# UCSD-Comp-Imaging/Nerf-Simple

Measured on AMD Instinct MI355X. Metric: ray-samples/sec at 800x800x128, higher is better.
Workload: dtype f16

## Files before the change

### nerf-simple_amd/csrc/dw_gemm.hip

```cpp
#include "nerf_device.h"

using namespace nerf_layout;

typedef __bf16 bf16x4 __attribute__((ext_vector_type(4)));

namespace {

constexpr int MAXD = 16;
struct GemmDesc {
    const __bf16* A;
    const __bf16* B;
    float* C;
    int lda, ldb, ldc;
    int M, N;
    int r0, Mv, Nv;
    int wg0, wgs;
    float* bias;
};
struct GemmTable {
    GemmDesc d[MAXD];
    int n;
    long long P;
};

constexpr int SLAB = 32;
static_assert(SLAB == 32, "the slab loop is written for two k-steps");
static_assert(ACT_TILE_PTS % SLAB == 0 && ACT_TILE_PTS * 16 == 4096, "a slab never straddles activation blocks");
constexpr int ROWB = 512;
constexpr int OPB = SLAB * ROWB;
constexpr int KSTEP = 16 * ROWB;
constexpr int SLOTB = 2 * OPB;
constexpr int RING = 4;
constexpr int LDS_BYTES = RING * SLOTB;
constexpr int DMA_PER_SLAB = 2 * SLAB / 2 / 8;

struct Frag { bf16x4 lo, hi; };
template <int KOFF>
__device__ __forceinline__ void read_frag_tr(Frag& f, unsigned addr_lo, unsigned addr_hi) {
    asm volatile("ds_read_b64_tr_b16 %0, %2 offset:%4\n\tds_read_b64_tr_b16 %1, %3 offset:%4"
                 : "=&v"(f.lo), "=&v"(f.hi) : "v"(addr_lo), "v"(addr_hi), "n"(KOFF));
}
__device__ __forceinline__ void frags_landed(Frag (&a)[4], Frag (&b)[2]) {
    asm volatile("s_waitcnt lgkmcnt(0)"
                 : "+v"(a[0].lo), "+v"(a[0].hi), "+v"(a[1].lo), "+v"(a[1].hi), "+v"(a[2].lo), "+v"(a[2].hi),
                   "+v"(a[3].lo), "+v"(a[3].hi), "+v"(b[0].lo), "+v"(b[0].hi), "+v"(b[1].lo), "+v"(b[1].hi));
}
__device__ __forceinline__ bf16x8 whole(const Frag& f) {
    return bf16x8{f.lo[0], f.lo[1], f.lo[2], f.lo[3], f.hi[0], f.hi[1], f.hi[2], f.hi[3]};
}

__global__ __launch_bounds__(512, 2) void dw_gemm_kernel(GemmTable tab) {
    extern __shared__ __attribute__((aligned(16))) char smem[];
    int di = 0;
    while (di + 1 < tab.n && (int)blockIdx.x >= tab.d[di + 1].wg0) ++di;
    const GemmDesc d = tab.d[di];
    const int slice = blockIdx.x - d.wg0;
    const long long nslab = (tab.P + SLAB - 1) / SLAB;
    const long long s_begin = nslab * slice / d.wgs, s_end = nslab * (slice + 1) / d.wgs;

    const int tid = threadIdx.x, lane = tid & 63;
    const int wave = __builtin_amdgcn_readfirstlane(tid >> 6);
    const int wm = wave >> 2, wn = wave & 3;
    const int m0 = 128 * wm, n0 = 64 * wn;

    const bool pieceA = wave < 4;
    const int pld = pieceA ? d.lda : d.ldb;
    const bool pblk = pld == 0;
    const __bf16* pbase = pieceA ? d.A : d.B;
    const int pwidth = pieceA ? d.M : d.N;
    const long long row_begin = s_begin * SLAB;
    const long long row_end = s_end * SLAB < tab.P ? s_end * SLAB : tab.P;
    const long long slice_rows = row_end > row_begin ? row_end - row_begin : 0;
    const long long slice_blocks = (row_end + ACT_TILE_PTS - 1) / ACT_TILE_PTS - row_begin / ACT_TILE_PTS;
    const __amdgpu_buffer_rsrc_t rs = pblk
        ? __builtin_amdgcn_make_buffer_rsrc(const_cast<char*>(reinterpret_cast<const char*>(pbase))
                                                + (row_begin / ACT_TILE_PTS) * ACT_BLOCK_BYTES,
                                            0, (int)(slice_rows > 0 ? slice_blocks * ACT_BLOCK_BYTES : 0), 0x00020000)
        : __builtin_amdgcn_make_buffer_rsrc(const_cast<__bf16*>(pbase + row_begin * pld), 0,
                                            (int)(slice_rows * pld * 2), 0x00020000);
    constexpr unsigned OUTSIDE = 0xffffffffu;
    unsigned voff[DMA_PER_SLAB];
    unsigned ldst[DMA_PER_SLAB];
    int vrow[DMA_PER_SLAB];
#pragma unroll
    for (int k = 0; k < DMA_PER_SLAB; ++k) {
        const int piece = wave * DMA_PER_SLAB + k, pi = piece & 15;
        ldst[k] = (piece >> 4) * OPB + pi * 1024;
        if (pblk) {
            const int c = 4 * (pi & 7) + (lane >> 4);
            vrow[k] = 16 * (pi >> 3) + ((lane & 15) ^ ((lane >> 4) << 2));
            voff[k] = c * 8 < pwidth ? (unsigned)(c * (ACT_TILE_PTS * 16) + vrow[k] * 16) : OUTSIDE;
        } else {
            vrow[k] = 2 * pi + (lane >> 5);
            const int cg = (lane & 31) ^ ((vrow[k] & 3) << 2);
            voff[k] = cg * 8 < pwidth ? (unsigned)(vrow[k] * pld * 2 + cg * 16) : OUTSIDE;
        }
    }
    auto issue_slab = [&](int it, int slot) {
        const long long p0 = row_begin + (long long)it * SLAB;
        unsigned vadd;
        int rows_left = SLAB;
        if (pblk) {
            vadd = (unsigned)((p0 / ACT_TILE_PTS - row_begin / ACT_TILE_PTS) * ACT_BLOCK_BYTES + (p0 % ACT_TILE_PTS) * 16);
            rows_left = tab.P - p0 < SLAB ? (int)(tab.P - p0) : SLAB;
        } else {
            vadd = (unsigned)it * (unsigned)(SLAB * pld * 2);
        }
#pragma unroll
        for (int k = 0; k < DMA_PER_SLAB; ++k) {
            lds_void* dst = reinterpret_cast<lds_void*>(reinterpret_cast<lds_char*>(0) + slot * SLOTB + ldst[k]);
            const unsigned off = (voff[k] == OUTSIDE || vrow[k] >= rows_left) ? OUTSIDE : voff[k] + vadd;
            __builtin_amdgcn_raw_ptr_buffer_load_lds(rs, dst, 16, off, 0, 0, 2);
        }
    };

    const int grp = lane >> 4, q = (lane & 15) >> 2, pp = lane & 3, h = lane >> 5;
    const int cl = 2 * (grp & 1) + (pp >> 1);
    auto frag_addr = [&](bool blocked, int t, int second) -> unsigned {
        const int r = 8 * h + q + 4 * second;
        if (blocked) return (4 * t + cl) * 256 + ((r ^ (cl << 2)) * 16) + 8 * (pp & 1);
        return r * ROWB + ((((4 * t + cl) ^ ((r & 3) << 2))) * 16) + 8 * (pp & 1);
    };
    unsigned aoff[4][2], boff[2][2];
#pragma unroll
    for (int i = 0; i < 4; ++i)
#pragma unroll
        for (int e = 0; e < 2; ++e) aoff[i][e] = frag_addr(d.lda == 0, m0 / 32 + i, e);
#pragma unroll
    for (int j = 0; j < 2; ++j)
#pragma unroll
        for (int e = 0; e < 2; ++e) boff[j][e] = OPB + frag_addr(d.ldb == 0, n0 / 32 + j, e);

    f32x16 acc[4][2];
#pragma unroll
    for (int i = 0; i < 4; ++i)
#pragma unroll
        for (int j = 0; j < 2; ++j)
#pragma unroll
            for (int r = 0; r < 16; ++r) acc[i][j][r] = 0.f;
    const bool active = m0 < d.M && n0 < d.N;
    float bsum[8] = {0.f, 0.f, 0.f, 0.f, 0.f, 0.f, 0.f, 0.f};
    const int brow = tid & 15, bchunk = tid >> 4;
    const unsigned baddr = bchunk * 256 + ((brow ^ ((bchunk & 3) << 2)) * 16);

#pragma unroll
    for (int k = 0; k < RING - 1; ++k)
        if (s_begin + k < s_end) issue_slab(k, k);
    Frag a0[4], b0[2], a1[4], b1[2];
    auto read_k0 = [&](unsigned base) {
#pragma unroll
        for (int i = 0; i < 4; ++i) read_frag_tr<0>(a0[i], base + aoff[i][0], base + aoff[i][1]);
#pragma unroll
        for (int j = 0; j < 2; ++j) read_frag_tr<0>(b0[j], base + boff[j][0], base + boff[j][1]);
    };
    if (s_begin < s_end) {
        const long long n = s_end - s_begin;
        if (n >= 3) asm volatile("s_waitcnt vmcnt(8)" ::: "memory");
        else if (n == 2) asm volatile("s_waitcnt vmcnt(4)" ::: "memory");
        else asm volatile("s_waitcnt vmcnt(0)" ::: "memory");
        __builtin_amdgcn_s_barrier();
        if (active) read_k0(0);
    }
    for (long long s = s_begin; s < s_end; ++s) {
        const int it = (int)(s - s_begin), slot = it & (RING - 1);
        const long long left = s_end - s;
        const unsigned base = slot * SLOTB;
        if (active) {
            frags_landed(a0, b0);
#pragma unroll
            for (int i = 0; i < 4; ++i) read_frag_tr<KSTEP>(a1[i], base + aoff[i][0], base + aoff[i][1]);
#pragma unroll
            for (int j = 0; j < 2; ++j) read_frag_tr<KSTEP>(b1[j], base + boff[j][0], base + boff[j][1]);
            __builtin_amdgcn_sched_barrier(0);
#pragma unroll
            for (int i = 0; i < 4; ++i)
#pragma unroll
                for (int j = 0; j < 2; ++j)
                    acc[i][j] = __builtin_amdgcn_mfma_f32_32x32x16_bf16(whole(a0[i]), whole(b0[j]), acc[i][j], 0, 0, 0);
            __builtin_amdgcn_sched_barrier(0);
        }
        if (left >= 2) {
            if (left >= 3) asm volatile("s_waitcnt vmcnt(4)" ::: "memory");
            else asm volatile("s_waitcnt vmcnt(0)" ::: "memory");
            __builtin_amdgcn_s_barrier();
            if (s + RING - 1 < s_end) issue_slab(it + RING - 1, (it + RING - 1) & (RING - 1));
        }
        if (active) {
            frags_landed(a1, b1);
            if (left >= 2) read_k0(((it + 1) & (RING - 1)) * SLOTB);
            __builtin_amdgcn_sched_barrier(0);
#pragma unroll
            for (int i = 0; i < 4; ++i)
#pragma unroll
                for (int j = 0; j < 2; ++j)
                    acc[i][j] = __builtin_amdgcn_mfma_f32_32x32x16_bf16(whole(a1[i]), whole(b1[j]), acc[i][j], 0, 0, 0);
        }
        if (d.bias && bchunk * 8 < d.M) {
#pragma unroll
            for (int ks = 0; ks < SLAB / 16; ++ks) {
                const bf16x8 v = *reinterpret_cast<const __attribute__((address_space(3))) bf16x8*>(
                    reinterpret_cast<lds_char*>(0) + base + ks * KSTEP + baddr);
#pragma unroll
                for (int k = 0; k < 8; ++k) bsum[k] += (float)v[k];
            }
        }
    }
    __syncthreads();
    if (d.bias && bchunk * 8 < d.M && s_begin < s_end) {
        float* red = reinterpret_cast<float*>(smem);
#pragma unroll
        for (int k = 0; k < 8; ++k) red[(brow * 32 + bchunk) * 8 + k] = bsum[k];
    }
    __syncthreads();
    if (d.bias && s_begin < s_end && tid < d.M) {
        const int ch = tid >> 3, k = tid & 7;
        float v = 0.f;
        for (int r = 0; r < 16; ++r) v += reinterpret_cast<float*>(smem)[(r * 32 + ch) * 8 + k];
        atomicAdd(d.bias + tid, v);
    }
    if (active && s_begin < s_end) {
#pragma unroll
        for (int i = 0; i < 4; ++i)
#pragma unroll
            for (int j = 0; j < 2; ++j)
#pragma unroll
                for (int r = 0; r < 16; ++r) {
                    const int row = m0 + 32 * i + (r & 3) + 8 * (r >> 2) + 4 * h - d.r0;
                    const int col = n0 + 32 * j + (lane & 31);
                    if (row >= 0 && row < d.Mv && col < d.Nv)
                        atomicAdd(d.C + (long long)row * d.ldc + col, acc[i][j][r]);
                }
    }
}

__global__ __launch_bounds__(256) void pack_draw_kernel(const float* __restrict__ d_raw, __bf16* __restrict__ dsr,
                                                        long long P, float* __restrict__ g_rgb_b,
                                                        float* __restrict__ g_sig_b) {
    __shared__ float red[4][4];
    f32x4 s = {0.f, 0.f, 0.f, 0.f};
    const __bf16 z = (__bf16)0.f;
    for (long long p = blockIdx.x * (long long)blockDim.x + threadIdx.x; p < P; p += (long long)gridDim.x * blockDim.x) {
        const f32x4 d = *reinterpret_cast<const f32x4*>(d_raw + p * 4);
        s += d;
        bf16x8* o = reinterpret_cast<bf16x8*>(dsr + p * 32);
        o[0] = bf16x8{(__bf16)d[0], (__bf16)d[1], (__bf16)d[2], (__bf16)d[3], z, z, z, z};
        o[1] = bf16x8{z, z, z, z, z, z, z, z};
        o[2] = o[1];
        o[3] = o[1];
    }
#pragma unroll
    for (int k = 0; k < 4; ++k) {
        float v = s[k];
#pragma unroll
        for (int off = 32; off >= 1; off >>= 1) v += __shfl_xor(v, off);
        if ((threadIdx.x & 63) == 0) red[threadIdx.x >> 6][k] = v;
    }
    __syncthreads();
    if (threadIdx.x < 4) {
        const float v = red[0][threadIdx.x] + red[1][threadIdx.x] + red[2][threadIdx.x] + red[3][threadIdx.x];
        atomicAdd(threadIdx.x < 3 ? g_rgb_b + threadIdx.x : g_sig_b, v);
    }
}

__global__ __launch_bounds__(256) void zero_f32_kernel(float* __restrict__ p, long long n) {
    const long long i = (blockIdx.x * (long long)blockDim.x + threadIdx.x) * 4;
    if (i + 3 < n) *reinterpret_cast<f32x4*>(p + i) = f32x4{0.f, 0.f, 0.f, 0.f};
    else for (long long k = i; k < n; ++k) p[k] = 0.f;
}

}

extern "C" int nerf_amd_launch_param_gradients_begin(const float* d_raw, void* scratch, float* grads, long long P,
                                                     hipStream_t stream) {
    (void)hipGetLastError();
    static_assert(PARAM_COUNT % 4 == 0, "16-byte zero fill");
    hipLaunchKernelGGL(zero_f32_kernel, dim3((PARAM_COUNT / 4 + 255) / 256), dim3(256), 0, stream, grads,
                       (long long)PARAM_COUNT);
    hipError_t e = hipGetLastError();
    if (e != hipSuccess) return (int)e;
    if (P <= 0) return 0;
    hipLaunchKernelGGL(pack_draw_kernel, dim3(512), dim3(256), 0, stream, d_raw, reinterpret_cast<__bf16*>(scratch), P,
                       grads + OFF_C1_B, grads + OFF_SIG_B);
    return (int)hipGetLastError();
}

extern "C" int nerf_amd_launch_param_gradients_finish(const void* acts_v, const void* dys_v, const void* posx64_v,
                                                      const void* posd32_v, const void* scratch, float* grads,
                                                      long long P, int bucket, hipStream_t stream) {
    (void)hipGetLastError();
    hipError_t e = hipSuccess;
    if (P <= 0) return 0;
    const __bf16* acts = reinterpret_cast<const __bf16*>(acts_v);
    const __bf16* dys = reinterpret_cast<const __bf16*>(dys_v);
    const __bf16* posx = reinterpret_cast<const __bf16*>(posx64_v);
    const __bf16* posd = reinterpret_cast<const __bf16*>(posd32_v);
    const __bf16* dsr = reinterpret_cast<const __bf16*>(scratch);
    auto act = [&](int L) { return acts + act_offset_bytes(L, P) / 2; };
    auto dy = [&](int L) { return dys + act_offset_bytes(L, P) / 2; };
    constexpr int BLK = 0;

    GemmTable t{};
    t.P = P;
    int n = 0;
    auto add = [&](const __bf16* A, int lda, int M, const __bf16* B, int ldb, int N, int coff, int ldc, int r0,
                   int Mv, int Nv, int boff = -1) {
        GemmDesc& g = t.d[n++];
        g.A = A; g.lda = lda; g.M = M; g.B = B; g.ldb = ldb; g.N = N;
        g.C = grads + coff; g.ldc = ldc; g.r0 = r0; g.Mv = Mv; g.Nv = Nv;
        g.bias = boff >= 0 ? grads + boff : nullptr;
    };
    const int LW = 256 * 256 + 256;
    add(dy(0), BLK, 256, posx, 64, 64, OFF_L0_W, 63, 0, 256, 63, OFF_L0_B);
    for (int l = 1; l <= 4; ++l)
        add(dy(l), BLK, 256, act(l - 1), BLK, 256, OFF_L1_W + (l - 1) * LW, 256, 0, 256, 256,
            OFF_L1_W + (l - 1) * LW + 65536);
    add(dy(5), BLK, 256, act(4), BLK, 256, OFF_SKIP_W, 319, 0, 256, 256, OFF_SKIP_B);
    add(dy(5), BLK, 256, posx, 64, 64, OFF_SKIP_W + 256, 319, 0, 256, 63);
    add(dy(6), BLK, 256, act(5), BLK, 256, OFF_L6_W, 256, 0, 256, 256, OFF_L6_W + 65536);
    add(dy(7), BLK, 256, act(6), BLK, 256, OFF_L6_W + LW, 256, 0, 256, 256, OFF_L6_W + LW + 65536);
    add(dsr, 32, 32, act(7), BLK, 256, OFF_SIG_W, 256, 3, 1, 256);
    add(dy(8), BLK, 256, act(7), BLK, 256, OFF_L2_W, 256, 0, 256, 256, OFF_L2_B);
    add(dy(9), BLK, 128, act(8), BLK, 256, OFF_C0_W, 283, 0, 128, 256, OFF_C0_B);
    add(dy(9), BLK, 128, posd, 32, 32, OFF_C0_W + 256, 283, 0, 128, 27);
    add(dsr, 32, 32, act(9), BLK, 128, OFF_C1_W, 128, 0, 3, 128);
    if (bucket != 0) {
        int m = 0;
        for (int i = 0; i < n; ++i) {
            const bool head = t.d[i].C - grads < GRAD_BUCKET_SPLIT;
            if (head == (bucket == 2)) t.d[m++] = t.d[i];
        }
        n = m;
    }
    t.n = n;
    constexpr double slab_cost = 1024.0;
    const int cus = device_cus();
    double total = 0;
    for (int i = 0; i < n; ++i) total += (double)(t.d[i].M + t.d[i].N) + slab_cost;
    const long long nslab = (P + SLAB - 1) / SLAB;
    const long long need = (P * 512 >> 30) + 1;
    long long w[16];
    double rem[16];
    long long used = 0;
    for (int i = 0; i < n; ++i) {
        const double share = ((double)(t.d[i].M + t.d[i].N) + slab_cost) / total * cus;
        w[i] = (long long)share;
        rem[i] = share - (double)w[i];
        if (w[i] < need) { w[i] = need; rem[i] = 0; }
        if (w[i] >= nslab) { w[i] = nslab; rem[i] = -1; }
        used += w[i];
    }
    while (used < cus) {
        int best = -1;
        for (int i = 0; i < n; ++i)
            if (rem[i] >= 0 && w[i] < nslab && (best < 0 || rem[i] > rem[best])) best = i;
        if (best < 0) break;
        ++w[best]; rem[best] = 0; ++used;
    }
    int wg = 0;
    for (int i = 0; i < n; ++i) {
        t.d[i].wg0 = wg;
        t.d[i].wgs = (int)w[i];
        wg += (int)w[i];
    }
    e = allow_dynamic_lds(reinterpret_cast<const void*>(dw_gemm_kernel), LDS_BYTES);
    if (e != hipSuccess) return (int)e;
    hipLaunchKernelGGL(dw_gemm_kernel, dim3(wg), dim3(512), LDS_BYTES, stream, t);

    return (int)hipGetLastError();
}

extern "C" int nerf_amd_launch_param_gradients(const float* d_raw, const void* acts_v, const void* dys_v,
                                               const void* posx64_v, const void* posd32_v, void* scratch,
                                               float* grads, long long P, hipStream_t stream) {
    const int rc = nerf_amd_launch_param_gradients_begin(d_raw, scratch, grads, P, stream);
    if (rc) return rc;
    return nerf_amd_launch_param_gradients_finish(acts_v, dys_v, posx64_v, posd32_v, scratch, grads, P, 0, stream);
}
```

### nerf-simple_amd/csrc/dw_gemm_f8.hip

```cpp
#include "nerf_device.h"

using namespace nerf_layout;

typedef int i32x8 __attribute__((ext_vector_type(8)));
typedef int i32x2 __attribute__((ext_vector_type(2)));

namespace {

constexpr int MAXD = 16;
struct F8Operand {
    const char* data;
    const unsigned char* scales;
    int block_bytes;
    int width;
};
struct GemmDescF8 {
    F8Operand A, B;
    float* C;
    int ldc;
    int r0, Mv, Nv;
    int wg0, wgs;
    float* bias;
};
struct GemmTableF8 {
    GemmDescF8 d[MAXD];
    int n;
    long long P;
};

constexpr int SLAB = 64;
constexpr int CHS = 1152;
constexpr int OPB = 16 * CHS;
constexpr int SLOTB = 2 * OPB;
constexpr int RING = 4;
constexpr int LDS_BYTES = RING * SLOTB;
constexpr int DMA_PER_SLAB = 4;
static_assert(ACT_TILE_PTS % SLAB == 0, "a slab never straddles tiles");

typedef __attribute__((address_space(4))) const u32x4 const_u32x4;

struct Frag { i32x2 q[4]; };
__device__ __forceinline__ void read_frag(Frag& f, unsigned addr) {
    asm volatile("ds_read_b64_tr_b8 %0, %4\n\tds_read_b64_tr_b8 %1, %4 offset:128\n\t"
                 "ds_read_b64_tr_b8 %2, %4 offset:512\n\tds_read_b64_tr_b8 %3, %4 offset:640"
                 : "=&v"(f.q[0]), "=&v"(f.q[1]), "=&v"(f.q[2]), "=&v"(f.q[3]) : "v"(addr));
}
__device__ __forceinline__ void frags_landed(Frag (&a)[4], Frag (&b)[2]) {
    asm volatile("s_waitcnt lgkmcnt(0)"
                 : "+v"(a[0].q[0]), "+v"(a[0].q[1]), "+v"(a[0].q[2]), "+v"(a[0].q[3]), "+v"(a[1].q[0]), "+v"(a[1].q[1]),
                   "+v"(a[1].q[2]), "+v"(a[1].q[3]), "+v"(a[2].q[0]), "+v"(a[2].q[1]), "+v"(a[2].q[2]), "+v"(a[2].q[3]),
                   "+v"(a[3].q[0]), "+v"(a[3].q[1]), "+v"(a[3].q[2]), "+v"(a[3].q[3]), "+v"(b[0].q[0]), "+v"(b[0].q[1]),
                   "+v"(b[0].q[2]), "+v"(b[0].q[3]), "+v"(b[1].q[0]), "+v"(b[1].q[1]), "+v"(b[1].q[2]), "+v"(b[1].q[3]));
}
__device__ __forceinline__ i32x8 whole(const Frag& f) {
    return i32x8{f.q[0][0], f.q[0][1], f.q[1][0], f.q[1][1], f.q[2][0], f.q[2][1], f.q[3][0], f.q[3][1]};
}
template <int OA, int OB>
__device__ __forceinline__ void mfma(const Frag& a, const Frag& b, f32x16& c, int sa, int sb) {
    const i32x8 av = whole(a), bv = whole(b);
    static_assert(OA >= 0 && OA < 4 && OB >= 0 && OB < 4, "op_sel picks one of four exponent bytes");
    asm volatile("v_mfma_scale_f32_32x32x64_f8f6f4 %0, %1, %2, %0, %3, %4 op_sel:[%5,%6,0] op_sel_hi:[%7,%8,0]"
                 : "+v"(c) : "v"(av), "v"(bv), "v"(sa), "v"(sb), "n"(OA & 1), "n"(OB & 1), "n"(OA >> 1), "n"(OB >> 1));
}

__global__ __launch_bounds__(512, 2) void dw_gemm_e4m3_kernel(GemmTableF8 tab) {
    extern __shared__ __attribute__((aligned(16))) char smem[];
    int di = 0;
    while (di + 1 < tab.n && (int)blockIdx.x >= tab.d[di + 1].wg0) ++di;
    const GemmDescF8 d = tab.d[di];
    const int slice = blockIdx.x - d.wg0;
    const long long nslab = (tab.P + SLAB - 1) / SLAB;
    const long long s_begin = nslab * slice / d.wgs, s_end = nslab * (slice + 1) / d.wgs;

    const int tid = threadIdx.x, lane = tid & 63;
    const int wave = __builtin_amdgcn_readfirstlane(tid >> 6);
    const int wm = wave >> 2, wn = wave & 3;
    const int m0 = 128 * wm, n0 = 64 * wn;
    const int M = d.A.width, N = d.B.width;

    const bool pieceA = wave < 4;
    const F8Operand op = pieceA ? d.A : d.B;
    const long long row_begin = s_begin * SLAB;
    const long long row_end = s_end * SLAB < tab.P ? s_end * SLAB : tab.P;
    const long long slice_rows = row_end > row_begin ? row_end - row_begin : 0;
    const long long tile0 = row_begin / ACT_TILE_PTS;
    const long long slice_tiles = (row_end + ACT_TILE_PTS - 1) / ACT_TILE_PTS - tile0;
    const __amdgpu_buffer_rsrc_t rs = __builtin_amdgcn_make_buffer_rsrc(
        const_cast<char*>(op.data) + tile0 * op.block_bytes, 0, (int)(slice_rows > 0 ? slice_tiles * op.block_bytes : 0), 0x00020000);
    constexpr unsigned OUTSIDE = 0xffffffffu;
    unsigned voff[DMA_PER_SLAB], ldst[DMA_PER_SLAB];
#pragma unroll
    for (int k = 0; k < DMA_PER_SLAB; ++k) {
        const int piece = wave * DMA_PER_SLAB + k, c = piece & 15;
        ldst[k] = (piece >> 4) * OPB + c * CHS;
        voff[k] = c * 16 < op.width ? (unsigned)(c * (ACT_TILE_PTS * 16) + lane * 16) : OUTSIDE;
    }
    auto issue_slab = [&](int it, int slot) {
        const long long p0 = row_begin + (long long)it * SLAB;
        const unsigned vadd = (unsigned)((p0 / ACT_TILE_PTS - tile0) * op.block_bytes + (p0 % ACT_TILE_PTS) * 16);
        const int rows_left = tab.P - p0 < SLAB ? (int)(tab.P - p0) : SLAB;
#pragma unroll
        for (int k = 0; k < DMA_PER_SLAB; ++k) {
            lds_void* dst = reinterpret_cast<lds_void*>(reinterpret_cast<lds_char*>(0) + slot * SLOTB + ldst[k]);
            const unsigned off = (voff[k] == OUTSIDE || lane >= rows_left) ? OUTSIDE : voff[k] + vadd;
            __builtin_amdgcn_raw_ptr_buffer_load_lds(rs, dst, 16, off, 0, 0, 2);
        }
    };

    const int h = lane >> 5;
    const unsigned lane_part = (unsigned)((16 * h + ((lane & 15) >> 1)) * 16 + (lane & 1) * 8 + ((lane >> 4) & 1) * CHS);
    unsigned aoff[4], boff[2];
#pragma unroll
    for (int i = 0; i < 4; ++i) aoff[i] = (unsigned)(2 * (m0 / 32 + i) * CHS) + lane_part;
#pragma unroll
    for (int j = 0; j < 2; ++j) boff[j] = OPB + (unsigned)(2 * (n0 / 32 + j) * CHS) + lane_part;

    f32x16 acc[4][2];
#pragma unroll
    for (int i = 0; i < 4; ++i)
#pragma unroll
        for (int j = 0; j < 2; ++j)
#pragma unroll
            for (int r = 0; r < 16; ++r) acc[i][j][r] = 0.f;
    const bool active = m0 < M && n0 < N;
    bool ta[4], tb[2];
#pragma unroll
    for (int i = 0; i < 4; ++i) ta[i] = active && m0 + 32 * i < M;
#pragma unroll
    for (int j = 0; j < 2; ++j) tb[j] = active && n0 + 32 * j < N;
    unsigned amask = 0, bmask = 0;
#pragma unroll
    for (int i = 0; i < 4; ++i) amask |= (m0 + 32 * i < M) ? 0xffu << (8 * i) : 0u;
#pragma unroll
    for (int j = 0; j < 2; ++j) bmask |= (n0 + 32 * j < N) ? 0xffu << (8 * j) : 0u;

    const bool do_bias = d.bias && m0 + 32 * wn < M;
    f32x16 accb;
#pragma unroll
    for (int r = 0; r < 16; ++r) accb[r] = 0.f;
    const unsigned aoff_bias = (unsigned)(2 * (m0 / 32 + wn) * CHS) + lane_part;
    Frag ab, ones;
#pragma unroll
    for (int q = 0; q < 4; ++q) ab.q[q] = i32x2{0, 0};
#pragma unroll
    for (int q = 0; q < 4; ++q) ones.q[q] = i32x2{0x38383838, 0x38383838};

    auto load_scales = [&](long long s, u32x4& ea, u32x4& eb) {
        const long long blk = s * (SLAB / 32);
        ea = *reinterpret_cast<const_u32x4*>(reinterpret_cast<uintptr_t>(d.A.scales + blk * 8));
        eb = *reinterpret_cast<const_u32x4*>(reinterpret_cast<uintptr_t>(d.B.scales + blk * 8));
    };

#pragma unroll
    for (int k = 0; k < RING - 1; ++k)
        if (s_begin + k < s_end) issue_slab(k, k);
    u32x4 ea = {0, 0, 0, 0}, eb = {0, 0, 0, 0};
    if (s_begin < s_end) load_scales(s_begin, ea, eb);

    Frag a[4], b[2];
    for (long long s = s_begin; s < s_end; ++s) {
        const int it = (int)(s - s_begin), slot = it & (RING - 1);
        const long long left = s_end - s;
        const unsigned base = slot * SLOTB;
        if (left >= 3) asm volatile("s_waitcnt vmcnt(8)" ::: "memory");
        else if (left == 2) asm volatile("s_waitcnt vmcnt(4)" ::: "memory");
        else asm volatile("s_waitcnt vmcnt(0)" ::: "memory");
        __builtin_amdgcn_s_barrier();
        if (s + RING - 1 < s_end) issue_slab(it + RING - 1, (it + RING - 1) & (RING - 1));
        const unsigned a_dw = (h ? (wm ? ea[3] : ea[2]) : (wm ? ea[1] : ea[0])) & amask;
        const unsigned b_dw = ((h ? ((wn >> 1) ? eb[3] : eb[2]) : ((wn >> 1) ? eb[1] : eb[0])) >> (16 * (wn & 1))) & bmask;
        const u32x4 ea_now = ea;
        if (left >= 2) load_scales(s + 1, ea, eb);
#if defined(F8_TIMING) && F8_TIMING == 4
        if (false) {
#else
        if (active || do_bias) {
#endif
            if (active) {
#pragma unroll
                for (int i = 0; i < 4; ++i) read_frag(a[i], base + aoff[i]);
#pragma unroll
                for (int j = 0; j < 2; ++j) read_frag(b[j], base + boff[j]);
            }
            if (do_bias) read_frag(ab, base + aoff_bias);
            frags_landed(a, b);
            asm volatile("" : "+v"(ab.q[0]), "+v"(ab.q[1]), "+v"(ab.q[2]), "+v"(ab.q[3]));
            __builtin_amdgcn_sched_barrier(0);
            if (ta[0] && tb[0]) mfma<0, 0>(a[0], b[0], acc[0][0], (int)a_dw, (int)b_dw);
            if (ta[0] && tb[1]) mfma<0, 1>(a[0], b[1], acc[0][1], (int)a_dw, (int)b_dw);
            if (ta[1] && tb[0]) mfma<1, 0>(a[1], b[0], acc[1][0], (int)a_dw, (int)b_dw);
            if (ta[1] && tb[1]) mfma<1, 1>(a[1], b[1], acc[1][1], (int)a_dw, (int)b_dw);
            if (ta[2] && tb[0]) mfma<2, 0>(a[2], b[0], acc[2][0], (int)a_dw, (int)b_dw);
            if (ta[2] && tb[1]) mfma<2, 1>(a[2], b[1], acc[2][1], (int)a_dw, (int)b_dw);
            if (ta[3] && tb[0]) mfma<3, 0>(a[3], b[0], acc[3][0], (int)a_dw, (int)b_dw);
            if (ta[3] && tb[1]) mfma<3, 1>(a[3], b[1], acc[3][1], (int)a_dw, (int)b_dw);
#if !(defined(F8_TIMING) && F8_TIMING == 5)
            if (do_bias) {
                constexpr int ONE = 0x7f7f7f7f;
                mfma<0, 0>(ab, ones, accb, (int)(a_dw >> (8 * wn)), ONE);
            }
#endif
        }
    }
    asm volatile("s_nop 15\n\ts_nop 15" ::: "memory");
    if (do_bias && s_begin < s_end && (lane & 31) == 0) {
#pragma unroll
        for (int r = 0; r < 16; ++r) {
            const int row = m0 + 32 * wn + (r & 3) + 8 * (r >> 2) + 4 * h;
            if (row < M) atomicAdd(d.bias + row, accb[r]);
        }
    }
    if (active && s_begin < s_end) {
#pragma unroll
        for (int i = 0; i < 4; ++i)
#pragma unroll
            for (int j = 0; j < 2; ++j)
#pragma unroll
                for (int r = 0; r < 16; ++r) {
                    const int row = m0 + 32 * i + (r & 3) + 8 * (r >> 2) + 4 * h - d.r0;
                    const int col = n0 + 32 * j + (lane & 31);
                    if (row >= 0 && row < d.Mv && col < d.Nv)
                        atomicAdd(d.C + (long long)row * d.ldc + col, acc[i][j][r]);
                }
    }
}

__global__ __launch_bounds__(256) void rows_to_e4m3_kernel(const __bf16* __restrict__ src, int ld, int W, long long P,
                                                           char* __restrict__ data, unsigned char* __restrict__ scales) {
    const int lane = threadIdx.x & 63;
    const int nq = (W + 31) / 32;
    const long long nblk = (P + 31) / 32;
    const long long wid = blockIdx.x * 4ll + (threadIdx.x >> 6);
    if (wid >= nblk * nq) return;
    const long long blk = wid / nq;
    const int Q = (int)(wid - blk * nq);
    const long long p = blk * 32 + (lane & 31);
    const int c = 2 * Q + (lane >> 5);
    const bool have = p < P && c * 16 < W;
    u32x4 w0 = {0, 0, 0, 0}, w1 = {0, 0, 0, 0};
    if (have) {
        const u32x4* sp = reinterpret_cast<const u32x4*>(src + p * ld + c * 16);
        w0 = sp[0];
        w1 = sp[1];
    }
    unsigned m = 0;
#pragma unroll
    for (int k = 0; k < 4; ++k) {
        const u16x2 x = __builtin_bit_cast(u16x2, w0[k] & 0x7fff7fffu), y = __builtin_bit_cast(u16x2, w1[k] & 0x7fff7fffu);
        m = __builtin_bit_cast(unsigned, __builtin_elementwise_max(__builtin_bit_cast(u16x2, m), __builtin_elementwise_max(x, y)));
    }
    unsigned mx = (m >> 16) > (m & 0xffffu) ? (m >> 16) : (m & 0xffffu);
#pragma unroll
    for (int off = 32; off >= 1; off >>= 1) {
        const unsigned o = (unsigned)__shfl_xor((int)mx, off);
        mx = o > mx ? o : mx;
    }
    const int e = (int)(mx >> 7);
    const int sb = e > 8 ? e - 7 : 1;
    const float scale = __builtin_bit_cast(float, sb << 23);
    s16x2 t = {0, 0};
    auto cvt = [&](unsigned lo, unsigned hi) -> unsigned {
        t = __builtin_amdgcn_cvt_scalef32_pk_fp8_bf16(t, __builtin_bit_cast(bf16x2, lo), scale, false);
        t = __builtin_amdgcn_cvt_scalef32_pk_fp8_bf16(t, __builtin_bit_cast(bf16x2, hi), scale, true);
        return __builtin_bit_cast(unsigned, t);
    };
    const u32x4 o = {cvt(w0[0], w0[1]), cvt(w0[2], w0[3]), cvt(w1[0], w1[1]), cvt(w1[2], w1[3])};
    if (have)
        *reinterpret_cast<u32x4*>(data + (p / ACT_TILE_PTS) * f8_narrow_block_bytes(W) + ((long long)c * ACT_TILE_PTS + p % ACT_TILE_PTS) * 16) = o;
    if (lane == 0) scales[blk * 8 + Q] = (unsigned char)sb;
}

}

static long long align256(long long v) { return (v + 255) / 256 * 256; }
extern "C" long long nerf_amd_f8_scratch_bytes(long long P) {
    return align256(f8_narrow_bytes(64, P)) + align256(f8_narrow_bytes(32, P)) + align256(f8_narrow_bytes(16, P));
}

extern "C" int nerf_amd_launch_param_gradients_convert_e4m3(const void* posx64_v, const void* posd32_v, const void* scratch,
                                                            void* scratch_f8, long long P, int which, hipStream_t stream) {
    (void)hipGetLastError();
    if (P <= 0) return 0;
    char* px = reinterpret_cast<char*>(scratch_f8);
    char* pd = px + align256(f8_narrow_bytes(64, P));
    char* ds = pd + align256(f8_narrow_bytes(32, P));
    const long long nblk = (P + 31) / 32;
    auto convert = [&](const void* src, int ld, int W, char* dst) {
        const long long waves = nblk * ((W + 31) / 32);
        hipLaunchKernelGGL(rows_to_e4m3_kernel, dim3((unsigned)((waves + 3) / 4)), dim3(256), 0, stream,
                           reinterpret_cast<const __bf16*>(src), ld, W, P, dst,
                           reinterpret_cast<unsigned char*>(dst + f8_narrow_scale_offset(W, P)));
    };
    if (which & 1) {
        convert(posx64_v, 64, 64, px);
        convert(posd32_v, 32, 32, pd);
    }
    if (which & 2) convert(scratch, 32, 16, ds);
    return (int)hipGetLastError();
}

extern "C" int nerf_amd_launch_param_gradients_finish_e4m3(const void* acts_v, const void* dys_v, const void* scratch_f8,
                                                           float* grads, long long P, int bucket, hipStream_t stream) {
    (void)hipGetLastError();
    if (P <= 0) return 0;
    hipError_t e = hipSuccess;
    const char* acts = reinterpret_cast<const char*>(acts_v);
    const char* dys = reinterpret_cast<const char*>(dys_v);
    const char* px = reinterpret_cast<const char*>(scratch_f8);
    const char* pd = px + align256(f8_narrow_bytes(64, P));
    const char* ds = pd + align256(f8_narrow_bytes(32, P));

    auto blocked = [&](const char* buf, int L) {
        return F8Operand{buf + f8_offset_bytes(L, P), reinterpret_cast<const unsigned char*>(buf + f8_scale_offset_bytes(L, P)),
                         (int)F8_BLOCK_BYTES, act_width(L)};
    };
    auto narrow = [&](const char* buf, int W) {
        return F8Operand{buf, reinterpret_cast<const unsigned char*>(buf + f8_narrow_scale_offset(W, P)), (int)f8_narrow_block_bytes(W), W};
    };
    GemmTableF8 t{};
    t.P = P;
    int n = 0;
    auto add = [&](F8Operand A, F8Operand B, int coff, int ldc, int r0, int Mv, int Nv, int boff = -1) {
        GemmDescF8& g = t.d[n++];
        g.A = A; g.B = B; g.C = grads + coff; g.ldc = ldc; g.r0 = r0; g.Mv = Mv; g.Nv = Nv;
        g.bias = boff >= 0 ? grads + boff : nullptr;
    };
    const int LW = 256 * 256 + 256;
    add(blocked(dys, 0), narrow(px, 64), OFF_L0_W, 63, 0, 256, 63, OFF_L0_B);
    for (int l = 1; l <= 4; ++l)
        add(blocked(dys, l), blocked(acts, l - 1), OFF_L1_W + (l - 1) * LW, 256, 0, 256, 256, OFF_L1_W + (l - 1) * LW + 65536);
    add(blocked(dys, 5), blocked(acts, 4), OFF_SKIP_W, 319, 0, 256, 256, OFF_SKIP_B);
    add(blocked(dys, 5), narrow(px, 64), OFF_SKIP_W + 256, 319, 0, 256, 63);
    add(blocked(dys, 6), blocked(acts, 5), OFF_L6_W, 256, 0, 256, 256, OFF_L6_W + 65536);
    add(blocked(dys, 7), blocked(acts, 6), OFF_L6_W + LW, 256, 0, 256, 256, OFF_L6_W + LW + 65536);
    add(narrow(ds, 16), blocked(acts, 7), OFF_SIG_W, 256, 3, 1, 256);
    add(blocked(dys, 8), blocked(acts, 7), OFF_L2_W, 256, 0, 256, 256, OFF_L2_B);
    add(blocked(dys, 9), blocked(acts, 8), OFF_C0_W, 283, 0, 128, 256, OFF_C0_B);
    add(blocked(dys, 9), narrow(pd, 32), OFF_C0_W + 256, 283, 0, 128, 27);
    add(narrow(ds, 16), blocked(acts, 9), OFF_C1_W, 128, 0, 3, 128);
    if (bucket != 0) {
        int m = 0;
        for (int i = 0; i < n; ++i) {
            const bool head = t.d[i].C - grads < GRAD_BUCKET_SPLIT;
            if (head == (bucket == 2)) t.d[m++] = t.d[i];
        }
        n = m;
    }
    t.n = n;
    constexpr double slab_cost = 1024.0;
    const int cus = device_cus();
    double total = 0;
    for (int i = 0; i < n; ++i) total += (double)(t.d[i].A.width + t.d[i].B.width) + slab_cost;
    const long long nslab = (P + SLAB - 1) / SLAB;
    const long long need = (P * 256 >> 30) + 1;
    long long w[16];
    double rem[16];
    long long used = 0;
    for (int i = 0; i < n; ++i) {
        const double share = ((double)(t.d[i].A.width + t.d[i].B.width) + slab_cost) / total * cus;
        w[i] = (long long)share;
        rem[i] = share - (double)w[i];
        if (w[i] < need) { w[i] = need; rem[i] = 0; }
        if (w[i] >= nslab) { w[i] = nslab; rem[i] = -1; }
        used += w[i];
    }
    while (used < cus) {
        int best = -1;
        for (int i = 0; i < n; ++i)
            if (rem[i] >= 0 && w[i] < nslab && (best < 0 || rem[i] > rem[best])) best = i;
        if (best < 0) break;
        ++w[best]; rem[best] = 0; ++used;
    }
    int wg = 0;
    for (int i = 0; i < n; ++i) {
        t.d[i].wg0 = wg;
        t.d[i].wgs = (int)w[i];
        wg += (int)w[i];
    }
    e = allow_dynamic_lds(reinterpret_cast<const void*>(dw_gemm_e4m3_kernel), LDS_BYTES);
    if (e != hipSuccess) return (int)e;
    hipLaunchKernelGGL(dw_gemm_e4m3_kernel, dim3(wg), dim3(512), LDS_BYTES, stream, t);
    return (int)hipGetLastError();
}
```

Before: 1.366 billion.

## Merge narrow side-product weight-gradient GEMMs into their wide sibling descriptors

Folds the thin weight-gradient products (sigma head and the direction-input half of color_fc.0) into the wide GEMM that shares an operand. The shared operand is then streamed once, and an extra narrow strip is loaded per slab into a new LDS region. In the bf16 kernel a spare wave or an extra MFMA chain handles the strip; in the f8 kernel wave 4 handles it. This removes separate descriptors, their workgroups and the repeated reads of the shared operand. In exchange the LDS footprint, the per-slab DMA count and the wait counts all grow, and the kernel gets extra branching, which may cut occupancy or lengthen the critical path.

```diff
diff --git a/nerf-simple_amd/csrc/dw_gemm.hip b/nerf-simple_amd/csrc/dw_gemm.hip
--- a/nerf-simple_amd/csrc/dw_gemm.hip
+++ b/nerf-simple_amd/csrc/dw_gemm.hip
@@ -16,6 +16,10 @@
     int r0, Mv, Nv;
     int wg0, wgs;
     float* bias;
+    const __bf16* X;
+    int xside;
+    float* XC;
+    int xldc, xr0, xMv, xNv;
 };
 struct GemmTable {
     GemmDesc d[MAXD];
@@ -27,12 +31,18 @@
 static_assert(SLAB == 32, "the slab loop is written for two k-steps");
 static_assert(ACT_TILE_PTS % SLAB == 0 && ACT_TILE_PTS * 16 == 4096, "a slab never straddles activation blocks");
 constexpr int ROWB = 512;
-constexpr int OPB = SLAB * ROWB;
-constexpr int KSTEP = 16 * ROWB;
-constexpr int SLOTB = 2 * OPB;
+constexpr int HALFB = 16 * ROWB;
+constexpr int XW = 32;
+constexpr int XROWB = XW * 2;
+constexpr int XHALFB = 16 * XROWB;
+constexpr int BOFF = HALFB, XOFF = 2 * HALFB;
+constexpr int KSTEP = 2 * HALFB + XHALFB;
+constexpr int SLOTB = 2 * KSTEP;
 constexpr int RING = 4;
 constexpr int LDS_BYTES = RING * SLOTB;
-constexpr int DMA_PER_SLAB = 2 * SLAB / 2 / 8;
+constexpr int WIDE_PER_SLAB = 2 * SLAB / 2 / 8;
+constexpr int DMA_PER_SLAB = WIDE_PER_SLAB + 1;
+static_assert(KSTEP % 256 == 0 && KSTEP < 65536 && LDS_BYTES <= 160 * 1024, "ds_read offset field; LDS of a CU");
 
 struct Frag { bf16x4 lo, hi; };
 template <int KOFF>
@@ -61,7 +71,9 @@
     const int tid = threadIdx.x, lane = tid & 63;
     const int wave = __builtin_amdgcn_readfirstlane(tid >> 6);
     const int wm = wave >> 2, wn = wave & 3;
-    const int m0 = 128 * wm, n0 = 64 * wn;
+    const bool xb = d.xside == 1 && wave == 4, xa = d.xside == 2;
+    const int m0 = xb ? 0 : 128 * wm, n0 = 64 * wn;
+    const int ct[2] = {xb ? 0 : n0 / 32 + wm, xb ? 1 : n0 / 32 + (wm ^ 1)};
 
     const bool pieceA = wave < 4;
     const int pld = pieceA ? d.lda : d.ldb;
@@ -79,13 +91,13 @@
         : __builtin_amdgcn_make_buffer_rsrc(const_cast<__bf16*>(pbase + row_begin * pld), 0,
                                             (int)(slice_rows * pld * 2), 0x00020000);
     constexpr unsigned OUTSIDE = 0xffffffffu;
-    unsigned voff[DMA_PER_SLAB];
-    unsigned ldst[DMA_PER_SLAB];
-    int vrow[DMA_PER_SLAB];
-#pragma unroll
-    for (int k = 0; k < DMA_PER_SLAB; ++k) {
-        const int piece = wave * DMA_PER_SLAB + k, pi = piece & 15;
-        ldst[k] = (piece >> 4) * OPB + pi * 1024;
+    unsigned voff[WIDE_PER_SLAB];
+    unsigned ldst[WIDE_PER_SLAB];
+    int vrow[WIDE_PER_SLAB];
+#pragma unroll
+    for (int k = 0; k < WIDE_PER_SLAB; ++k) {
+        const int piece = wave * WIDE_PER_SLAB + k, pi = piece & 15;
+        ldst[k] = (pi >> 3) * KSTEP + (piece >> 4) * HALFB + (pi & 7) * 1024;
         if (pblk) {
             const int c = 4 * (pi & 7) + (lane >> 4);
             vrow[k] = 16 * (pi >> 3) + ((lane & 15) ^ ((lane >> 4) << 2));
@@ -96,6 +108,10 @@
             voff[k] = cg * 8 < pwidth ? (unsigned)(vrow[k] * pld * 2 + cg * 16) : OUTSIDE;
         }
     }
+    const __amdgpu_buffer_rsrc_t rsx = __builtin_amdgcn_make_buffer_rsrc(
+        const_cast<__bf16*>(d.X ? d.X + row_begin * XW : d.A), 0, (int)(d.X ? slice_rows * XROWB : 0), 0x00020000);
+    const unsigned xvoff = (unsigned)(wave * 4 * XROWB + lane * 16);
+    const unsigned xldst = (wave >> 2) * KSTEP + XOFF + (wave & 3) * 4 * XROWB;
     auto issue_slab = [&](int it, int slot) {
         const long long p0 = row_begin + (long long)it * SLAB;
         unsigned vadd;
@@ -107,10 +123,14 @@
             vadd = (unsigned)it * (unsigned)(SLAB * pld * 2);
         }
 #pragma unroll
-        for (int k = 0; k < DMA_PER_SLAB; ++k) {
+        for (int k = 0; k < WIDE_PER_SLAB; ++k) {
             lds_void* dst = reinterpret_cast<lds_void*>(reinterpret_cast<lds_char*>(0) + slot * SLOTB + ldst[k]);
             const unsigned off = (voff[k] == OUTSIDE || vrow[k] >= rows_left) ? OUTSIDE : voff[k] + vadd;
             __builtin_amdgcn_raw_ptr_buffer_load_lds(rs, dst, 16, off, 0, 0, 2);
+        }
+        if (lane < 16) {
+            lds_void* dst = reinterpret_cast<lds_void*>(reinterpret_cast<lds_char*>(0) + slot * SLOTB + xldst);
+            __builtin_amdgcn_raw_ptr_buffer_load_lds(rsx, dst, 16, xvoff + (unsigned)it * (unsigned)(SLAB * XROWB), 0, 0, 2);
         }
     };
 
@@ -121,7 +141,9 @@
         if (blocked) return (4 * t + cl) * 256 + ((r ^ (cl << 2)) * 16) + 8 * (pp & 1);
         return r * ROWB + ((((4 * t + cl) ^ ((r & 3) << 2))) * 16) + 8 * (pp & 1);
     };
-    unsigned aoff[4][2], boff[2][2];
+    unsigned aoff[4][2], boff[2][2], xoff[2];
+#pragma unroll
+    for (int e = 0; e < 2; ++e) xoff[e] = XOFF + (8 * h + q + 4 * e) * XROWB + cl * 16 + 8 * (pp & 1);
 #pragma unroll
     for (int i = 0; i < 4; ++i)
 #pragma unroll
@@ -129,7 +151,7 @@
 #pragma unroll
     for (int j = 0; j < 2; ++j)
 #pragma unroll
-        for (int e = 0; e < 2; ++e) boff[j][e] = OPB + frag_addr(d.ldb == 0, n0 / 32 + j, e);
+        for (int e = 0; e < 2; ++e) boff[j][e] = xb ? xoff[e] : BOFF + frag_addr(d.ldb == 0, ct[j], e);
 
     f32x16 acc[4][2];
 #pragma unroll
@@ -138,7 +160,10 @@
         for (int j = 0; j < 2; ++j)
 #pragma unroll
             for (int r = 0; r < 16; ++r) acc[i][j][r] = 0.f;
-    const bool active = m0 < d.M && n0 < d.N;
+    f32x16 accx;
+#pragma unroll
+    for (int r = 0; r < 16; ++r) accx[r] = 0.f;
+    const bool active = xb || (m0 < d.M && n0 < d.N);
     float bsum[8] = {0.f, 0.f, 0.f, 0.f, 0.f, 0.f, 0.f, 0.f};
     const int brow = tid & 15, bchunk = tid >> 4;
     const unsigned baddr = bchunk * 256 + ((brow ^ ((bchunk & 3) << 2)) * 16);
@@ -146,8 +171,10 @@
 #pragma unroll
     for (int k = 0; k < RING - 1; ++k)
         if (s_begin + k < s_end) issue_slab(k, k);
-    Frag a0[4], b0[2], a1[4], b1[2];
+    Frag a0[4], b0[2], a1[4], b1[2], ax0, ax1;
+    ax0.lo = ax0.hi = ax1.lo = ax1.hi = bf16x4{(__bf16)0.f, (__bf16)0.f, (__bf16)0.f, (__bf16)0.f};
     auto read_k0 = [&](unsigned base) {
+        if (xa) read_frag_tr<0>(ax0, base + xoff[0], base + xoff[1]);
 #pragma unroll
         for (int i = 0; i < 4; ++i) read_frag_tr<0>(a0[i], base + aoff[i][0], base + aoff[i][1]);
 #pragma unroll
@@ -155,8 +182,8 @@
     };
     if (s_begin < s_end) {
         const long long n = s_end - s_begin;
-        if (n >= 3) asm volatile("s_waitcnt vmcnt(8)" ::: "memory");
-        else if (n == 2) asm volatile("s_waitcnt vmcnt(4)" ::: "memory");
+        if (n >= 3) asm volatile("s_waitcnt vmcnt(%0)" :: "n"(2 * DMA_PER_SLAB) : "memory");
+        else if (n == 2) asm volatile("s_waitcnt vmcnt(%0)" :: "n"(DMA_PER_SLAB) : "memory");
         else asm volatile("s_waitcnt vmcnt(0)" ::: "memory");
         __builtin_amdgcn_s_barrier();
         if (active) read_k0(0);
@@ -167,6 +194,8 @@
         const unsigned base = slot * SLOTB;
         if (active) {
             frags_landed(a0, b0);
+            asm volatile("" : "+v"(ax0.lo), "+v"(ax0.hi));
+            if (xa) read_frag_tr<KSTEP>(ax1, base + xoff[0], base + xoff[1]);
 #pragma unroll
             for (int i = 0; i < 4; ++i) read_frag_tr<KSTEP>(a1[i], base + aoff[i][0], base + aoff[i][1]);
 #pragma unroll
@@ -177,16 +206,18 @@
 #pragma unroll
                 for (int j = 0; j < 2; ++j)
                     acc[i][j] = __builtin_amdgcn_mfma_f32_32x32x16_bf16(whole(a0[i]), whole(b0[j]), acc[i][j], 0, 0, 0);
+            if (xa) accx = __builtin_amdgcn_mfma_f32_32x32x16_bf16(whole(ax0), whole(b0[0]), accx, 0, 0, 0);
             __builtin_amdgcn_sched_barrier(0);
         }
         if (left >= 2) {
-            if (left >= 3) asm volatile("s_waitcnt vmcnt(4)" ::: "memory");
+            if (left >= 3) asm volatile("s_waitcnt vmcnt(%0)" :: "n"(DMA_PER_SLAB) : "memory");
             else asm volatile("s_waitcnt vmcnt(0)" ::: "memory");
             __builtin_amdgcn_s_barrier();
             if (s + RING - 1 < s_end) issue_slab(it + RING - 1, (it + RING - 1) & (RING - 1));
         }
         if (active) {
             frags_landed(a1, b1);
+            asm volatile("" : "+v"(ax1.lo), "+v"(ax1.hi));
             if (left >= 2) read_k0(((it + 1) & (RING - 1)) * SLOTB);
             __builtin_amdgcn_sched_barrier(0);
 #pragma unroll
@@ -194,6 +225,7 @@
 #pragma unroll
                 for (int j = 0; j < 2; ++j)
                     acc[i][j] = __builtin_amdgcn_mfma_f32_32x32x16_bf16(whole(a1[i]), whole(b1[j]), acc[i][j], 0, 0, 0);
+            if (xa) accx = __builtin_amdgcn_mfma_f32_32x32x16_bf16(whole(ax1), whole(b1[0]), accx, 0, 0, 0);
         }
         if (d.bias && bchunk * 8 < d.M) {
 #pragma unroll
@@ -219,17 +251,28 @@
         atomicAdd(d.bias + tid, v);
     }
     if (active && s_begin < s_end) {
+        float* const C = xb ? d.XC : d.C;
+        const int ldc = xb ? d.xldc : d.ldc, r0 = xb ? d.xr0 : d.r0, Mv = xb ? d.xMv : d.Mv, Nv = xb ? d.xNv : d.Nv;
 #pragma unroll
         for (int i = 0; i < 4; ++i)
 #pragma unroll
             for (int j = 0; j < 2; ++j)
 #pragma unroll
                 for (int r = 0; r < 16; ++r) {
-                    const int row = m0 + 32 * i + (r & 3) + 8 * (r >> 2) + 4 * h - d.r0;
-                    const int col = n0 + 32 * j + (lane & 31);
-                    if (row >= 0 && row < d.Mv && col < d.Nv)
-                        atomicAdd(d.C + (long long)row * d.ldc + col, acc[i][j][r]);
+                    const int row = m0 + 32 * i + (r & 3) + 8 * (r >> 2) + 4 * h - r0;
+                    const int col = 32 * ct[j] + (lane & 31);
+                    if (row >= 0 && row < Mv && col < Nv)
+                        atomicAdd(C + (long long)row * ldc + col, acc[i][j][r]);
                 }
+        if (xa) {
+#pragma unroll
+            for (int r = 0; r < 16; ++r) {
+                const int row = (r & 3) + 8 * (r >> 2) + 4 * h - d.xr0;
+                const int col = 32 * ct[0] + (lane & 31);
+                if (row >= 0 && row < d.xMv && col < d.xNv && col < d.N)
+                    atomicAdd(d.XC + (long long)row * d.xldc + col, accx[r]);
+            }
+        }
     }
 }
 
@@ -309,6 +352,12 @@
         g.C = grads + coff; g.ldc = ldc; g.r0 = r0; g.Mv = Mv; g.Nv = Nv;
         g.bias = boff >= 0 ? grads + boff : nullptr;
     };
+    auto merge = [&](int side, const __bf16* X, int coff, int ldc, int r0, int Mv, int Nv) {
+        GemmDesc& g = t.d[n - 1];
+        g.X = X; g.xside = side; g.XC = grads + coff; g.xldc = ldc; g.xr0 = r0; g.xMv = Mv; g.xNv = Nv;
+    };
+    static_assert(OFF_SIG_W >= GRAD_BUCKET_SPLIT && OFF_L2_W >= GRAD_BUCKET_SPLIT && OFF_C0_W >= GRAD_BUCKET_SPLIT,
+                  "layers_2 + sigma_fc.0 and both halves of color_fc.0 are late-bucket tensors");
     const int LW = 256 * 256 + 256;
     add(dy(0), BLK, 256, posx, 64, 64, OFF_L0_W, 63, 0, 256, 63, OFF_L0_B);
     for (int l = 1; l <= 4; ++l)
@@ -318,10 +367,10 @@
     add(dy(5), BLK, 256, posx, 64, 64, OFF_SKIP_W + 256, 319, 0, 256, 63);
     add(dy(6), BLK, 256, act(5), BLK, 256, OFF_L6_W, 256, 0, 256, 256, OFF_L6_W + 65536);
     add(dy(7), BLK, 256, act(6), BLK, 256, OFF_L6_W + LW, 256, 0, 256, 256, OFF_L6_W + LW + 65536);
-    add(dsr, 32, 32, act(7), BLK, 256, OFF_SIG_W, 256, 3, 1, 256);
     add(dy(8), BLK, 256, act(7), BLK, 256, OFF_L2_W, 256, 0, 256, 256, OFF_L2_B);
+    merge(2, dsr, OFF_SIG_W, 256, 3, 1, 256);
     add(dy(9), BLK, 128, act(8), BLK, 256, OFF_C0_W, 283, 0, 128, 256, OFF_C0_B);
-    add(dy(9), BLK, 128, posd, 32, 32, OFF_C0_W + 256, 283, 0, 128, 27);
+    merge(1, posd, OFF_C0_W + 256, 283, 0, 128, 27);
     add(dsr, 32, 32, act(9), BLK, 128, OFF_C1_W, 128, 0, 3, 128);
     if (bucket != 0) {
         int m = 0;
@@ -335,14 +384,15 @@
     constexpr double slab_cost = 1024.0;
     const int cus = device_cus();
     double total = 0;
-    for (int i = 0; i < n; ++i) total += (double)(t.d[i].M + t.d[i].N) + slab_cost;
+    auto width = [&](const GemmDesc& g) { return (double)(g.M + g.N + (g.X ? XW : 0)); };
+    for (int i = 0; i < n; ++i) total += width(t.d[i]) + slab_cost;
     const long long nslab = (P + SLAB - 1) / SLAB;
     const long long need = (P * 512 >> 30) + 1;
     long long w[16];
     double rem[16];
     long long used = 0;
     for (int i = 0; i < n; ++i) {
-        const double share = ((double)(t.d[i].M + t.d[i].N) + slab_cost) / total * cus;
+        const double share = (width(t.d[i]) + slab_cost) / total * cus;
         w[i] = (long long)share;
         rem[i] = share - (double)w[i];
         if (w[i] < need) { w[i] = need; rem[i] = 0; }
diff --git a/nerf-simple_amd/csrc/dw_gemm_f8.hip b/nerf-simple_amd/csrc/dw_gemm_f8.hip
--- a/nerf-simple_amd/csrc/dw_gemm_f8.hip
+++ b/nerf-simple_amd/csrc/dw_gemm_f8.hip
@@ -21,6 +21,9 @@
     int r0, Mv, Nv;
     int wg0, wgs;
     float* bias;
+    F8Operand X;
+    float* XC;
+    int xldc, xr0, xMv, xNv;
 };
 struct GemmTableF8 {
     GemmDescF8 d[MAXD];
@@ -31,10 +34,13 @@
 constexpr int SLAB = 64;
 constexpr int CHS = 1152;
 constexpr int OPB = 16 * CHS;
-constexpr int SLOTB = 2 * OPB;
+constexpr int XOFF = 2 * OPB;
+constexpr int SLOTB = 2 * OPB + 2 * CHS;
 constexpr int RING = 4;
 constexpr int LDS_BYTES = RING * SLOTB;
-constexpr int DMA_PER_SLAB = 4;
+constexpr int WIDE_PER_SLAB = 4;
+constexpr int DMA_PER_SLAB = WIDE_PER_SLAB + 1;
+static_assert(LDS_BYTES <= 160 * 1024, "LDS of a CU");
 static_assert(ACT_TILE_PTS % SLAB == 0, "a slab never straddles tiles");
 
 typedef __attribute__((address_space(4))) const u32x4 const_u32x4;
@@ -75,8 +81,10 @@
     const int tid = threadIdx.x, lane = tid & 63;
     const int wave = __builtin_amdgcn_readfirstlane(tid >> 6);
     const int wm = wave >> 2, wn = wave & 3;
-    const int m0 = 128 * wm, n0 = 64 * wn;
-    const int M = d.A.width, N = d.B.width;
+    const bool xb = d.X.data != nullptr && wave == 4;
+    const int mb = 128 * wm;
+    const int m0 = xb ? 0 : mb, n0 = 64 * wn;
+    const int M = d.A.width, N = xb ? 32 : d.B.width;
 
     const bool pieceA = wave < 4;
     const F8Operand op = pieceA ? d.A : d.B;
@@ -88,23 +96,34 @@
     const __amdgpu_buffer_rsrc_t rs = __builtin_amdgcn_make_buffer_rsrc(
         const_cast<char*>(op.data) + tile0 * op.block_bytes, 0, (int)(slice_rows > 0 ? slice_tiles * op.block_bytes : 0), 0x00020000);
     constexpr unsigned OUTSIDE = 0xffffffffu;
-    unsigned voff[DMA_PER_SLAB], ldst[DMA_PER_SLAB];
-#pragma unroll
-    for (int k = 0; k < DMA_PER_SLAB; ++k) {
-        const int piece = wave * DMA_PER_SLAB + k, c = piece & 15;
+    unsigned voff[WIDE_PER_SLAB], ldst[WIDE_PER_SLAB];
+#pragma unroll
+    for (int k = 0; k < WIDE_PER_SLAB; ++k) {
+        const int piece = wave * WIDE_PER_SLAB + k, c = piece & 15;
         ldst[k] = (piece >> 4) * OPB + c * CHS;
         voff[k] = c * 16 < op.width ? (unsigned)(c * (ACT_TILE_PTS * 16) + lane * 16) : OUTSIDE;
     }
+    const int xblock = d.X.data ? d.X.block_bytes : 0;
+    const __amdgpu_buffer_rsrc_t rsx = __builtin_amdgcn_make_buffer_rsrc(
+        const_cast<char*>(d.X.data ? d.X.data + tile0 * xblock : op.data), 0, (int)(slice_rows > 0 ? slice_tiles * xblock : 0), 0x00020000);
+    const int xpt = 16 * (wave & 3) + lane;
+    const unsigned xvoff = (unsigned)((wave >> 2) * (ACT_TILE_PTS * 16) + xpt * 16);
+    const unsigned xldst = XOFF + (wave >> 2) * CHS + (wave & 3) * 256;
     auto issue_slab = [&](int it, int slot) {
         const long long p0 = row_begin + (long long)it * SLAB;
         const unsigned vadd = (unsigned)((p0 / ACT_TILE_PTS - tile0) * op.block_bytes + (p0 % ACT_TILE_PTS) * 16);
         const int rows_left = tab.P - p0 < SLAB ? (int)(tab.P - p0) : SLAB;
 #pragma unroll
-        for (int k = 0; k < DMA_PER_SLAB; ++k) {
+        for (int k = 0; k < WIDE_PER_SLAB; ++k) {
             lds_void* dst = reinterpret_cast<lds_void*>(reinterpret_cast<lds_char*>(0) + slot * SLOTB + ldst[k]);
             const unsigned off = (voff[k] == OUTSIDE || lane >= rows_left) ? OUTSIDE : voff[k] + vadd;
             __builtin_amdgcn_raw_ptr_buffer_load_lds(rs, dst, 16, off, 0, 0, 2);
         }
+        if (lane < 16) {
+            lds_void* dst = reinterpret_cast<lds_void*>(reinterpret_cast<lds_char*>(0) + slot * SLOTB + xldst);
+            const unsigned xvadd = (unsigned)((p0 / ACT_TILE_PTS - tile0) * xblock + (p0 % ACT_TILE_PTS) * 16);
+            __builtin_amdgcn_raw_ptr_buffer_load_lds(rsx, dst, 16, xpt >= rows_left ? OUTSIDE : xvoff + xvadd, 0, 0, 2);
+        }
     };
 
     const int h = lane >> 5;
@@ -113,7 +132,7 @@
 #pragma unroll
     for (int i = 0; i < 4; ++i) aoff[i] = (unsigned)(2 * (m0 / 32 + i) * CHS) + lane_part;
 #pragma unroll
-    for (int j = 0; j < 2; ++j) boff[j] = OPB + (unsigned)(2 * (n0 / 32 + j) * CHS) + lane_part;
+    for (int j = 0; j < 2; ++j) boff[j] = (xb ? XOFF : OPB + (unsigned)(2 * (n0 / 32) * CHS)) + (unsigned)(2 * j * CHS) + lane_part;
 
     f32x16 acc[4][2];
 #pragma unroll
@@ -134,21 +153,23 @@
 #pragma unroll
     for (int j = 0; j < 2; ++j) bmask |= (n0 + 32 * j < N) ? 0xffu << (8 * j) : 0u;
 
-    const bool do_bias = d.bias && m0 + 32 * wn < M;
+    const bool do_bias = d.bias && mb + 32 * wn < M;
     f32x16 accb;
 #pragma unroll
     for (int r = 0; r < 16; ++r) accb[r] = 0.f;
-    const unsigned aoff_bias = (unsigned)(2 * (m0 / 32 + wn) * CHS) + lane_part;
+    const unsigned aoff_bias = (unsigned)(2 * (mb / 32 + wn) * CHS) + lane_part;
     Frag ab, ones;
 #pragma unroll
     for (int q = 0; q < 4; ++q) ab.q[q] = i32x2{0, 0};
 #pragma unroll
     for (int q = 0; q < 4; ++q) ones.q[q] = i32x2{0x38383838, 0x38383838};
 
+    const unsigned char* const bscales = xb ? d.X.scales : d.B.scales;
+    const int wma = xb ? 0 : wm;
     auto load_scales = [&](long long s, u32x4& ea, u32x4& eb) {
         const long long blk = s * (SLAB / 32);
         ea = *reinterpret_cast<const_u32x4*>(reinterpret_cast<uintptr_t>(d.A.scales + blk * 8));
-        eb = *reinterpret_cast<const_u32x4*>(reinterpret_cast<uintptr_t>(d.B.scales + blk * 8));
+        eb = *reinterpret_cast<const_u32x4*>(reinterpret_cast<uintptr_t>(bscales + blk * 8));
     };
 
 #pragma unroll
@@ -162,12 +183,12 @@
         const int it = (int)(s - s_begin), slot = it & (RING - 1);
         const long long left = s_end - s;
         const unsigned base = slot * SLOTB;
-        if (left >= 3) asm volatile("s_waitcnt vmcnt(8)" ::: "memory");
-        else if (left == 2) asm volatile("s_waitcnt vmcnt(4)" ::: "memory");
+        if (left >= 3) asm volatile("s_waitcnt vmcnt(%0)" :: "n"(2 * DMA_PER_SLAB) : "memory");
+        else if (left == 2) asm volatile("s_waitcnt vmcnt(%0)" :: "n"(DMA_PER_SLAB) : "memory");
         else asm volatile("s_waitcnt vmcnt(0)" ::: "memory");
         __builtin_amdgcn_s_barrier();
         if (s + RING - 1 < s_end) issue_slab(it + RING - 1, (it + RING - 1) & (RING - 1));
-        const unsigned a_dw = (h ? (wm ? ea[3] : ea[2]) : (wm ? ea[1] : ea[0])) & amask;
+        const unsigned a_dw = (h ? (wma ? ea[3] : ea[2]) : (wma ? ea[1] : ea[0])) & amask;
         const unsigned b_dw = ((h ? ((wn >> 1) ? eb[3] : eb[2]) : ((wn >> 1) ? eb[1] : eb[0])) >> (16 * (wn & 1))) & bmask;
         const u32x4 ea_now = ea;
         if (left >= 2) load_scales(s + 1, ea, eb);
@@ -206,21 +227,23 @@
     if (do_bias && s_begin < s_end && (lane & 31) == 0) {
 #pragma unroll
         for (int r = 0; r < 16; ++r) {
-            const int row = m0 + 32 * wn + (r & 3) + 8 * (r >> 2) + 4 * h;
+            const int row = mb + 32 * wn + (r & 3) + 8 * (r >> 2) + 4 * h;
             if (row < M) atomicAdd(d.bias + row, accb[r]);
         }
     }
     if (active && s_begin < s_end) {
+        float* const C = xb ? d.XC : d.C;
+        const int ldc = xb ? d.xldc : d.ldc, r0 = xb ? d.xr0 : d.r0, Mv = xb ? d.xMv : d.Mv, Nv = xb ? d.xNv : d.Nv;
 #pragma unroll
         for (int i = 0; i < 4; ++i)
 #pragma unroll
             for (int j = 0; j < 2; ++j)
 #pragma unroll
                 for (int r = 0; r < 16; ++r) {
-                    const int row = m0 + 32 * i + (r & 3) + 8 * (r >> 2) + 4 * h - d.r0;
+                    const int row = m0 + 32 * i + (r & 3) + 8 * (r >> 2) + 4 * h - r0;
                     const int col = n0 + 32 * j + (lane & 31);
-                    if (row >= 0 && row < d.Mv && col < d.Nv)
-                        atomicAdd(d.C + (long long)row * d.ldc + col, acc[i][j][r]);
+                    if (row >= 0 && row < Mv && col < Nv && col < N)
+                        atomicAdd(C + (long long)row * ldc + col, acc[i][j][r]);
                 }
     }
 }
@@ -325,6 +348,11 @@
         g.A = A; g.B = B; g.C = grads + coff; g.ldc = ldc; g.r0 = r0; g.Mv = Mv; g.Nv = Nv;
         g.bias = boff >= 0 ? grads + boff : nullptr;
     };
+    auto merge = [&](F8Operand X, int coff, int ldc, int r0, int Mv, int Nv) {
+        GemmDescF8& g = t.d[n - 1];
+        g.X = X; g.XC = grads + coff; g.xldc = ldc; g.xr0 = r0; g.xMv = Mv; g.xNv = Nv;
+    };
+    static_assert(OFF_C0_W >= GRAD_BUCKET_SPLIT, "both halves of color_fc.0 lie in the late bucket (the filter goes by the fat product)");
     const int LW = 256 * 256 + 256;
     add(blocked(dys, 0), narrow(px, 64), OFF_L0_W, 63, 0, 256, 63, OFF_L0_B);
     for (int l = 1; l <= 4; ++l)
@@ -336,7 +364,7 @@
     add(narrow(ds, 16), blocked(acts, 7), OFF_SIG_W, 256, 3, 1, 256);
     add(blocked(dys, 8), blocked(acts, 7), OFF_L2_W, 256, 0, 256, 256, OFF_L2_B);
     add(blocked(dys, 9), blocked(acts, 8), OFF_C0_W, 283, 0, 128, 256, OFF_C0_B);
-    add(blocked(dys, 9), narrow(pd, 32), OFF_C0_W + 256, 283, 0, 128, 27);
+    merge(narrow(pd, 32), OFF_C0_W + 256, 283, 0, 128, 27);
     add(narrow(ds, 16), blocked(acts, 9), OFF_C1_W, 128, 0, 3, 128);
     if (bucket != 0) {
         int m = 0;
@@ -350,14 +378,15 @@
     constexpr double slab_cost = 1024.0;
     const int cus = device_cus();
     double total = 0;
-    for (int i = 0; i < n; ++i) total += (double)(t.d[i].A.width + t.d[i].B.width) + slab_cost;
+    auto width = [&](const GemmDescF8& g) { return (double)(g.A.width + g.B.width + (g.X.data ? g.X.width : 0)); };
+    for (int i = 0; i < n; ++i) total += width(t.d[i]) + slab_cost;
     const long long nslab = (P + SLAB - 1) / SLAB;
     const long long need = (P * 256 >> 30) + 1;
     long long w[16];
     double rem[16];
     long long used = 0;
     for (int i = 0; i < n; ++i) {
-        const double share = ((double)(t.d[i].A.width + t.d[i].B.width) + slab_cost) / total * cus;
+        const double share = (width(t.d[i]) + slab_cost) / total * cus;
         w[i] = (long long)share;
         rem[i] = share - (double)w[i];
         if (w[i] < need) { w[i] = need; rem[i] = 0; }
```

Result: no change. 1.362 billion (-0.3%).
